# kylejckson/PaintFE

Measured on AMD Instinct MI355X. Metric: Mpixels/sec: 8K 32-layer flatten + Gaussian sigma=16; HBM GB/s vs peak, higher is better.
Workload: dtype f32 (Gaussian leg: f16 taps x u8, f32 accumulate)

## Files before the change

paintfe_amd/csrc/k_flatten.hip:

```cpp
#include <algorithm>
#include <atomic>
#include <type_traits>
#include "k_common.h"
#include "pfx_kernels.h"

using namespace pfxk;

#include "k_blend.h"

typedef float pfx_v4f __attribute__((ext_vector_type(4)));
typedef int pfx_v4i __attribute__((ext_vector_type(4)));
__device__ pfx_v4f pfx_buffer_load_format_v4f32(pfx_v4i rsrc, int voffset, int soffset, int aux) __asm("llvm.amdgcn.raw.buffer.load.format.v4f32");
__device__ float pfx_buffer_load_format_f32(pfx_v4i rsrc, int voffset, int soffset, int aux) __asm("llvm.amdgcn.raw.buffer.load.format.f32");
__device__ void pfx_buffer_store_i32(int data, pfx_v4i rsrc, int voffset, int soffset, int aux) __asm("llvm.amdgcn.raw.buffer.store.i32");
__device__ void pfx_buffer_store_format_v4f32(pfx_v4f data, pfx_v4i rsrc, int voffset, int soffset, int aux) __asm("llvm.amdgcn.raw.buffer.store.format.v4f32");


namespace {


PFX_DEV uint32_t apply_conceal(uint32_t px, uint32_t conceal)
{
    if (conceal == 0u) return px;
    uint32_t a = ((px >> 24) * (255u - conceal)) / 255u;
// ... 464 lines not shown
                    }
                }
                if (lane == 0) { rec[u % NREC][0] = r; rec[u % NREC][1] = best != 0u ? q_tail : 0u; }
                wave_lds_sync();
                cls_next = u + 1u;
                continue;
            }
            if (q_cnt == 0u) {
                if (lane == 0 && (C.stats & 1u)) {
                    atomicAdd(&g_dle_stats[0], st_rounds); atomicAdd(&g_dle_stats[1], st_rpx); atomicAdd(&g_dle_stats[2], st_rlay);
                    atomicAdd(&g_dle_stats[3], nat_next); atomicAdd(&g_dle_stats[4], st_nlay); atomicAdd(&g_dle_stats[5], st_reads);
                    atomicAdd(&g_dle_stats[6], st_cunits);
                }
                break;
            }
            run_queue = true;
        }

        int voff[PX];
        float acc[PX][4];
        uint32_t lb, le;
        if (run_queue) {
            const uint32_t m = min(q_cnt, UPX);
#pragma unroll
            for (int j = 0; j < PX; ++j) {
                const uint32_t k = 64u * j + lane;
                const uint32_t o = (uint32_t)q[(q_head + k) % QCAP];
                voff[j] = k < m ? (int)((base_px + o) * 4u) : (int)bytes;
                acc[j][0] = acc[j][1] = acc[j][2] = acc[j][3] = 0.0f;
            }
            lb = q_start; le = q_r;
            q_head += m;
            st_rounds += 1u; st_rpx += m; st_rlay += le - lb;
        } else {
            const uint32_t o0 = nat_next * UPX + lane;
#pragma unroll
            for (int j = 0; j < PX; ++j) {
                voff[j] = (int)((base_px + o0 + 64u * j) * 4u);
                const uint32_t p = acc_ring[(o0 + 64u * j) % RING];
                acc[j][0] = div255(ubyte0(p)); acc[j][1] = div255(ubyte1(p)); acc[j][2] = div255(ubyte2(p)); acc[j][3] = div255(ubyte3(p));
            }
            lb = nat_start; le = n_layers;
            st_nlay += le - lb;
        }
        dle_layers<PX, NB, AUX>(acc, layers, lb, le, bytes, voff, (C.stats & 2u) != 0u);
#pragma unroll
        for (int j = 0; j < PX; ++j) {
            const uint32_t px = (uint32_t)(acc[j][0] * 255.0f + 0.5f) | ((uint32_t)(acc[j][1] * 255.0f + 0.5f) << 8) |
                                ((uint32_t)(acc[j][2] * 255.0f + 0.5f) << 16) | ((uint32_t)(acc[j][3] * 255.0f + 0.5f) << 24);
            if (run_queue) { if (voff[j] != (int)bytes) acc_ring[((uint32_t)voff[j] / 4u - base_px) % RING] = px; }
            else pfx_buffer_store_i32((int)px, rs_dst, voff[j], 0, 0);
        }
        if (run_queue) wave_lds_sync();
        else nat_next += 1u;
    }
}


#ifndef PFX_SRT_GROUPS
#define PFX_SRT_GROUPS 1
#endif
#ifndef PFX_SRT_REDEAL
#define PFX_SRT_REDEAL 1
#endif
#ifndef PFX_SRT_TYPED_STORE
#define PFX_SRT_TYPED_STORE 0
#endif
#ifndef PFX_SRT_NATSTORE
#define PFX_SRT_NATSTORE 1
#endif
template <int PX>
PFX_DEV void stream_layer_groups(float (&acc)[PX][4], const float (&t)[PX][4], uint32_t mode, float opacity, uint32_t lead)
{
    const float amax = alpha_max<PX>(t);
#if PFX_TWO_STAGE
    if (__any(amax != 0.0f)) blend_layer_nx_two_stage<PX>(mode, acc, t, opacity, lead);
#elif PFX_SRT_GROUPS
    if (__any(amax != 0.0f)) blend_layer_nx_groups<PX>(mode, acc, t, opacity, lead);
#else
    if (__any(amax != 0.0f)) blend_layer_nx<PX>(mode, acc, t, opacity);
#endif
}

template <int PX, bool NOBLEND = false, bool TR = false>
PFX_DEV void srt_layers(float (&acc)[PX][4], const pfxk_layer_desc* __restrict__ layers, uint32_t lb, uint32_t le, uint32_t bytes, int (&voff)[PX],
                        uint32_t s1, uint32_t seg, float4* s_x, uint32_t* s_v, uint32_t& st_moves, unsigned long long* tr = nullptr)
{
    float t[2][PX][4];
    uint32_t m[2], o[2];
    const pfxk_layer_desc* nptr = layers + lb;
    pfxk_layer_desc nd = *nptr;
    uint32_t next_attempt = lb < s1 ? s1 : lb + 1u;
    uint32_t lead = 0u;
    bool recount = true;
    auto fetch = [&](auto SET) {
        constexpr int S = decltype(SET)::value;
        m[S] = nd.mode; o[S] = nd.adj_off;
        const pfx_v4i rs = make_rsrc_canonical(nd.pixels, bytes, PFX_RSRC_UNORM8X4);
#pragma unroll
        for (int j = 0; j < PX; ++j) {
            const pfx_v4f v = pfx_buffer_load_format_v4f32(rs, voff[j], 0, 0);
            t[S][j][0] = v.x; t[S][j][1] = v.y; t[S][j][2] = v.z; t[S][j][3] = v.w;
        }
        nptr += 1;
        nd = *nptr;
    };
    auto blend = [&](auto SET, uint32_t K) {
        constexpr int S = decltype(SET)::value;
        if (K < le) {
            unsigned long long c0 = 0, c1 = 0;
            if constexpr (TR) {
                c0 = __builtin_amdgcn_s_memtime();
                if constexpr (PX == 1) asm volatile("s_waitcnt vmcnt(1)" ::: "memory");
                else if constexpr (PX == 2) asm volatile("s_waitcnt vmcnt(2)" ::: "memory");
                else asm volatile("s_waitcnt vmcnt(3)" ::: "memory");
                c1 = __builtin_amdgcn_s_memtime();
                tr[0] += c1 - c0;
            }
            if constexpr (NOBLEND) {
#pragma unroll
                for (int j = 0; j < PX; ++j) { acc[j][0] += t[S][j][0]; acc[j][1] += t[S][j][1]; acc[j][2] += t[S][j][2]; acc[j][3] = t[S][j][3]; }
            } else if constexpr (PX == 1 && !PFX_TWO_STAGE) {
                stream_layer<1>(acc, t[S], m[S], __builtin_bit_cast(float, __builtin_amdgcn_readfirstlane(o[S])));
            } else {
                if (recount) { lead = count_lead<PX>(acc); recount = false; }
                stream_layer_groups<PX>(acc, t[S], m[S], __builtin_bit_cast(float, __builtin_amdgcn_readfirstlane(o[S])), lead);
                recount = m[S] == M_XOR || m[S] == M_OVERWRITE;
            }
            if constexpr (TR) {
                float sink = 0.0f;
#pragma unroll
                for (int j = 0; j < PX; ++j) sink += acc[j][0] + acc[j][3];
                asm volatile("" :: "v"(sink));
                tr[1] += __builtin_amdgcn_s_memtime() - c1;
            }
        }
    };
    auto redeal = [&](auto SET, uint32_t K) {
        constexpr int S = decltype(SET)::value;
#if !PFX_SRT_REDEAL
        return;
#endif
        if constexpr (PX == 1 || NOBLEND) return;
        if (K != next_attempt || K >= le) return;
        next_attempt = K + seg;
        uint64_t mo[PX];
        uint32_t co[PX], total_o = 0u, now = 0u;
        bool run = true;
#pragma unroll
        for (int j = 0; j < PX; ++j) {
            mo[j] = __ballot(acc[j][3] == 1.0f);
            co[j] = (uint32_t)__popcll(mo[j]);
            total_o += co[j];
            run = run && co[j] == 64u;
            now += run ? 1u : 0u;
        }
        lead = now; recount = false;
        if (total_o / 64u <= now) return;
        lead = total_o / 64u;
        const uint32_t lane = __builtin_amdgcn_mbcnt_hi(~0u, __builtin_amdgcn_mbcnt_lo(~0u, 0u));
        uint32_t slot[PX], pre_o = 0u, pre_n = total_o;
#pragma unroll
        for (int j = 0; j < PX; ++j) {
            const uint32_t rank_o = __builtin_amdgcn_mbcnt_hi((uint32_t)(mo[j] >> 32), __builtin_amdgcn_mbcnt_lo((uint32_t)mo[j], 0u));
            slot[j] = acc[j][3] == 1.0f ? pre_o + rank_o : pre_n + (lane - rank_o);
            pre_o += co[j]; pre_n += 64u - co[j];
        }
#pragma unroll
        for (int j = 0; j < PX; ++j) { s_x[slot[j]] = make_float4(acc[j][0], acc[j][1], acc[j][2], acc[j][3]); s_v[slot[j]] = (uint32_t)voff[j]; }
        wave_lds_sync();
#pragma unroll
        for (int j = 0; j < PX; ++j) {
            const float4 a = s_x[64u * j + lane];
            acc[j][0] = a.x; acc[j][1] = a.y; acc[j][2] = a.z; acc[j][3] = a.w;
            voff[j] = (int)s_v[64u * j + lane];
        }
        wave_lds_sync();
#pragma unroll
        for (int j = 0; j < PX; ++j) s_x[slot[j]] = make_float4(t[S][j][0], t[S][j][1], t[S][j][2], t[S][j][3]);
        wave_lds_sync();
#pragma unroll
        for (int j = 0; j < PX; ++j) {
            const float4 a = s_x[64u * j + lane];
            t[S][j][0] = a.x; t[S][j][1] = a.y; t[S][j][2] = a.z; t[S][j][3] = a.w;
        }
        wave_lds_sync();
        st_moves += 1u;
    };
    fetch(std::integral_constant<int, 0>{});
    for (uint32_t li = lb; li < le; li += 2) {
        fetch(std::integral_constant<int, 1>{}); blend(std::integral_constant<int, 0>{}, li); redeal(std::integral_constant<int, 1>{}, li + 1);
        fetch(std::integral_constant<int, 0>{}); blend(std::integral_constant<int, 1>{}, li + 1); redeal(std::integral_constant<int, 0>{}, li + 2);
    }
}

template <int NB, bool NOBLEND = false, bool TR = false>
PFX_DEV void srt_early(float (&acc)[1][4], const pfxk_layer_desc* __restrict__ layers, uint32_t lb, uint32_t le, uint32_t bytes, int voff, unsigned long long* tr = nullptr)
{
    static_assert(NB >= 2 && 2 * NB - 2 < PFXK_DESC_PAD, "descriptor padding");
    float t[NB][1][4];
    uint32_t m[NB], o[NB];
    const pfxk_layer_desc* nptr = layers + lb;
    pfxk_layer_desc nd = *nptr;
    uint32_t lead = 0u;
    bool recount = true;
    auto fetch = [&](auto SET) {
        constexpr int S = decltype(SET)::value;
        m[S] = nd.mode; o[S] = nd.adj_off;
        const pfx_v4i rs = make_rsrc_canonical(nd.pixels, bytes, PFX_RSRC_UNORM8X4);
        const pfx_v4f v = pfx_buffer_load_format_v4f32(rs, voff, 0, 0);
        t[S][0][0] = v.x; t[S][0][1] = v.y; t[S][0][2] = v.z; t[S][0][3] = v.w;
        nptr += 1;
        nd = *nptr;
    };
    auto blend = [&](auto SET, uint32_t K) {
        constexpr int S = decltype(SET)::value;
        if (K < le) {
            unsigned long long c0 = 0, c1 = 0;
            if constexpr (TR) {
                c0 = __builtin_amdgcn_s_memtime();
                asm volatile("s_waitcnt vmcnt(%0)" :: "n"(NB - 1) : "memory");
                c1 = __builtin_amdgcn_s_memtime();
                tr[0] += c1 - c0;
            }
            if constexpr (NOBLEND) { acc[0][0] += t[S][0][0]; acc[0][1] += t[S][0][1]; acc[0][2] += t[S][0][2]; acc[0][3] = t[S][0][3]; }
            else {
                if (recount) { lead = count_lead<1>(acc); recount = false; }
                stream_layer_groups<1>(acc, t[S], m[S], __builtin_bit_cast(float, __builtin_amdgcn_readfirstlane(o[S])), lead);
                recount = true;
            }
            if constexpr (TR) {
                const float sink = acc[0][0] + acc[0][3];
                asm volatile("" :: "v"(sink));
                tr[1] += __builtin_amdgcn_s_memtime() - c1;
            }
        }
    };
    auto seq = [&](auto self, auto I, uint32_t li) {
        constexpr int i = decltype(I)::value;
        if constexpr (i < NB) {
            fetch(std::integral_constant<int, (i + NB - 1) % NB>{});
            blend(std::integral_constant<int, i>{}, li + (uint32_t)i);
            self(self, std::integral_constant<int, i + 1>{}, li);
        }
    };
    auto pre = [&](auto self, auto I) {
        constexpr int i = decltype(I)::value;
        if constexpr (i < NB - 1) { fetch(std::integral_constant<int, i>{}); self(self, std::integral_constant<int, i + 1>{}); }
    };
    pre(pre, std::integral_constant<int, 0>{});
    for (uint32_t li = lb; li < le; li += (uint32_t)NB) seq(seq, std::integral_constant<int, 0>{}, li);
}
#ifndef PFX_EARLY_NB
#define PFX_EARLY_NB 2
#endif

struct dle_plan { uint32_t s1, seg; };

#ifndef PFX_SRT_PRIO
#define PFX_SRT_PRIO 0
#endif
#ifndef PFX_SRT_WAVES
#define PFX_SRT_WAVES 8
#endif
#if PFX_SRT_WAVES == 8
#define PFX_SRT_ATTR __attribute__((amdgpu_waves_per_eu(8, 8)))
#elif PFX_SRT_WAVES == 7
#define PFX_SRT_ATTR __attribute__((amdgpu_waves_per_eu(7, 7)))
#else
#define PFX_SRT_ATTR
#endif
template <int PX, bool NOBLEND = false, bool TR = false>
__global__ __launch_bounds__(64) PFX_SRT_ATTR void flatten_srt_kernel(const pfxk_layer_desc* __restrict__ layers, uint32_t n_layers, uint32_t n_px,
                                                                         uint8_t* __restrict__ dst, const pfxk_dle_cands C, const dle_sched SC,
                                                                         const dle_plan P)
{
    constexpr uint32_t UPX = 64u * PX;
    __shared__ float4 s_x[UPX];
    __shared__ uint32_t s_v[UPX];
    soft_d_fill(threadIdx.x, 64u);
    __syncthreads();
    const uint32_t lane = threadIdx.x & 63u;
    const uint32_t gw = __builtin_amdgcn_readfirstlane(blockIdx.x);
    const uint32_t units_total = (n_px + UPX - 1u) / UPX;
    uint32_t u0, U;
    if (gw < SC.wavesA) { U = SC.UA; u0 = gw * SC.UA; }
    else if (gw < SC.wavesA + SC.wavesB) { U = SC.UB; u0 = SC.wavesA * SC.UA + (gw - SC.wavesA) * SC.UB; }
    else { U = SC.UC; u0 = SC.wavesA * SC.UA + SC.wavesB * SC.UB + (gw - SC.wavesA - SC.wavesB) * SC.UC; }
    if (u0 >= units_total) return;
    const uint32_t nu = min(U, units_total - u0);
    const uint32_t base_px = u0 * UPX;
    const uint32_t bytes = n_px * 4u;
#if PFX_SRT_TYPED_STORE
    const pfx_v4i rs_acc = make_rsrc(dst, bytes, PFX_RSRC_UNORM8X4);
#else
    const pfx_v4i rs_dst = make_rsrc(dst, bytes, PFX_RSRC_RAW32);
#endif
    const uint32_t s1 = P.seg != 0u ? P.s1 : 0xFFFFFFFFu;
    uint32_t st_egroups = 0, st_elay = 0, st_nlay = 0, st_reads = 0, st_cunits = 0, st_moves = 0;
    uint32_t probe_fail = 0, skip_left = 0;
    unsigned long long tph[8] = {0, 0, 0, 0, 0, 0, 0, 0}, tc0 = 0;
    const unsigned long long t_birth = TR ? __builtin_amdgcn_s_memtime() : 0ull;
    for (uint32_t u = 0; u < nu; ++u) {
        if constexpr (TR) tc0 = __builtin_amdgcn_s_memtime();
        int voff[PX];
        float acc[PX][4];
#pragma unroll
        for (int j = 0; j < PX; ++j) {
            voff[j] = (int)((base_px + u * UPX + 64u * j + lane) * 4u);
            acc[j][0] = acc[j][1] = acc[j][2] = acc[j][3] = 0.0f;
        }
        uint32_t cls[PX];
#pragma unroll
        for (int j = 0; j < PX; ++j) cls[j] = 0u;
        const bool probe = skip_left == 0u;
        if (!probe) skip_left -= 1u;
        bool done = !probe;
#pragma unroll
        for (int i = 3; i >= 0; --i) {
            if ((uint32_t)i < C.n && !done) {
                const pfx_v4i ra = make_rsrc(layers[C.layer[i]].pixels, bytes, PFX_RSRC_ALPHA8);
                bool all_found = true;
#pragma unroll
                for (int j = 0; j < PX; ++j) {
                    const float a = pfx_buffer_load_format_f32(ra, voff[j], 0, 0);
                    const bool hit = C.kind[i] ? (a == 1.0f) : (a != 0.0f);
                    cls[j] = (cls[j] == 0u && hit) ? (uint32_t)(i + 1) : cls[j];
                    all_found = all_found && cls[j] != 0u;
                }
                done = __all(all_found);
                st_reads += 1u;
            }
        }
        uint32_t cn[5] = {UPX, 0u, 0u, 0u, 0u};
#pragma unroll
        for (int i = 1; i <= 4; ++i)
#pragma unroll
            for (int j = 0; j < PX; ++j) cn[i] += (uint32_t)__popcll(__ballot(cls[j] >= (uint32_t)i));
        uint32_t cmin = 0;
#pragma unroll
        for (int i = 1; i <= 4; ++i) if (cn[i] == UPX) cmin = (uint32_t)i;
        const uint32_t lay[5] = {0u, C.layer[0], C.layer[1], C.layer[2], C.layer[3]};
        uint32_t s_u = 0;
#pragma unroll
        for (int i = 1; i <= 4; ++i) if (cmin == (uint32_t)i) s_u = lay[i];
        uint32_t best = 0, best_sav = 0, r = s_u, eg = 0, cn_best = 0;
#pragma unroll
        for (int i = 1; i <= 4; ++i) {
            if ((uint32_t)i > cmin && (uint32_t)i <= C.n) {
                const uint32_t g = (UPX - cn[i] + 63u) / 64u;
                const uint32_t sav = ((uint32_t)PX - g) * (lay[i] - s_u);
                if (sav > best_sav) { best_sav = sav; best = (uint32_t)i; r = lay[i]; eg = g; cn_best = cn[i]; }
            }
        }
        if (probe) {
            if (best != 0u || s_u != 0u) probe_fail = 0u;
            else if (++probe_fail >= 2u) { probe_fail = 0u; skip_left = 14u; }
        }
        if constexpr (TR) { const unsigned long long c = __builtin_amdgcn_s_memtime(); tph[0] += c - tc0; tc0 = c; }
        if (best != 0u) {
            st_cunits += 1u;
            uint32_t pre_e = 0u, pre_l = UPX - cn_best;
#pragma unroll
            for (int j = 0; j < PX; ++j) {
                const bool early = cls[j] < best;
                const uint64_t m = __ballot(early);
                const uint32_t rank_e = __builtin_amdgcn_mbcnt_hi((uint32_t)(m >> 32), __builtin_amdgcn_mbcnt_lo((uint32_t)m, 0u));
                const uint32_t c = (uint32_t)__popcll(m);
                s_v[early ? pre_e + rank_e : pre_l + (lane - rank_e)] = (uint32_t)voff[j];
                pre_e += c; pre_l += 64u - c;
            }
            wave_lds_sync();
#pragma unroll
            for (int j = 0; j < PX; ++j) voff[j] = (int)s_v[64u * j + lane];
            wave_lds_sync();
            for (uint32_t g = 0; g < eg; ++g) {
                int v1[1];
                float a1[1][4] = {{0.0f, 0.0f, 0.0f, 0.0f}};
                v1[0] = voff[0];
#pragma unroll
                for (int j = 1; j < PX; ++j) v1[0] = g == (uint32_t)j ? voff[j] : v1[0];
                uint32_t none = 0u;
#if PFX_SRT_PRIO
                __builtin_amdgcn_s_setprio(PFX_SRT_PRIO & 3);
#endif
#if PFX_EARLY_NB > 0
                (void)none;
                srt_early<PFX_EARLY_NB, NOBLEND, TR>(a1, layers, s_u, r, bytes, v1[0], tph + 4);
#else
                srt_layers<1, NOBLEND, TR>(a1, layers, s_u, r, bytes, v1, 0xFFFFFFFFu, 0u, s_x, s_v, none, tph + 4);
#endif
#pragma unroll
                for (int j = 0; j < PX; ++j)
                    if (g == (uint32_t)j) { acc[j][0] = a1[0][0]; acc[j][1] = a1[0][1]; acc[j][2] = a1[0][2]; acc[j][3] = a1[0][3]; }
            }
            st_egroups += eg; st_elay += eg * (r - s_u);
        }
        st_nlay += n_layers - r;
        const uint32_t moves_before = st_moves;
        if constexpr (TR) { const unsigned long long c = __builtin_amdgcn_s_memtime(); tph[1] += c - tc0; tc0 = c; }
#if PFX_SRT_PRIO
        __builtin_amdgcn_s_setprio((PFX_SRT_PRIO >> 2) & 3);
#endif
        srt_layers<PX, NOBLEND, TR>(acc, layers, r, n_layers, bytes, voff, s1, P.seg, s_x, s_v, st_moves, tph + 6);
        if constexpr (TR) { const unsigned long long c = __builtin_amdgcn_s_memtime(); tph[2] += c - tc0; tc0 = c; }
        if (PFX_SRT_NATSTORE && (best != 0u || st_moves != moves_before)) {
            const uint32_t ub = (base_px + u * UPX) * 4u;
#pragma unroll
            for (int j = 0; j < PX; ++j) s_x[((uint32_t)voff[j] - ub) >> 2] = make_float4(acc[j][0], acc[j][1], acc[j][2], acc[j][3]);
            wave_lds_sync();
#pragma unroll
            for (int j = 0; j < PX; ++j) {
                const float4 a = s_x[64u * j + lane];
                acc[j][0] = a.x; acc[j][1] = a.y; acc[j][2] = a.z; acc[j][3] = a.w;
                voff[j] = (int)(ub + (64u * j + lane) * 4u);
            }
            wave_lds_sync();
        }
#pragma unroll
        for (int j = 0; j < PX; ++j) {
#if PFX_SRT_TYPED_STORE
            pfx_v4f v; v.x = acc[j][0]; v.y = acc[j][1]; v.z = acc[j][2]; v.w = acc[j][3];
            pfx_buffer_store_format_v4f32(v, rs_acc, voff[j], 0, 0);
#else
            uint32_t px = 0u;
#pragma unroll
            for (int c = 0; c < 4; ++c) px = __builtin_amdgcn_cvt_pk_u8_f32(acc[j][c] * 255.0f, c, px);
            pfx_buffer_store_i32((int)px, rs_dst, voff[j], 0, 0);
#endif
        }
        if constexpr (TR) { const unsigned long long c = __builtin_amdgcn_s_memtime(); tph[3] += c - tc0; tc0 = c; }
    }
    if constexpr (TR) {
        if (lane == 0) {
#pragma unroll
            for (int i = 0; i < 8; ++i) atomicAdd(&g_dle_stats[8 + i], tph[i]);
            atomicAdd(&g_dle_stats[0], __builtin_amdgcn_s_memtime() - t_birth);
            atomicAdd(&g_dle_stats[1], 1ull);
        }
        return;
    }
    if (lane == 0 && (C.stats & 1u)) {
        atomicAdd(&g_dle_stats[0], st_egroups); atomicAdd(&g_dle_stats[1], st_egroups * 64u); atomicAdd(&g_dle_stats[2], st_elay);
        atomicAdd(&g_dle_stats[3], nu); atomicAdd(&g_dle_stats[4], st_nlay); atomicAdd(&g_dle_stats[5], st_reads);
        atomicAdd(&g_dle_stats[6], st_cunits); atomicAdd(&g_dle_stats[7], st_moves);
    }
}

__global__ __launch_bounds__(1024) void dle_probe_kernel(const pfxk_layer_desc* __restrict__ layers, uint32_t cand_layer, uint32_t cand_kind, uint32_t n_px,
                                                         uint32_t* __restrict__ verdict_pinned, uint32_t tag)
{
    __shared__ uint32_t s_cnt;
    if (threadIdx.x == 0) s_cnt = 0u;
    __syncthreads();
    const uint32_t lane = threadIdx.x & 63u, wave = threadIdx.x >> 6;
    const uint32_t units = (n_px + 191u) / 192u, bytes = n_px * 4u;
    const pfx_v4i ra = make_rsrc(layers[cand_layer].pixels, bytes, PFX_RSRC_ALPHA8);
    uint32_t good = 0u;
#pragma unroll 4
    for (uint32_t k = 0; k < 16u; ++k) {
        const uint32_t u = (uint32_t)(((uint64_t)(wave * 16u + k) * units) / 256u);
        bool all_hit = true;
#pragma unroll
        for (uint32_t j = 0; j < 3u; ++j) {
            const uint32_t px = u * 192u + 64u * j + lane;
            const float a = pfx_buffer_load_format_f32(ra, (int)(px * 4u), 0, 0);
            all_hit = all_hit && (px >= n_px || (cand_kind ? (a == 1.0f) : (a != 0.0f)));
        }
        good += __all(all_hit) ? 1u : 0u;
    }
    if (lane == 0) atomicAdd(&s_cnt, good);
    __syncthreads();
    if (threadIdx.x == 0) *verdict_pinned = tag | (s_cnt * 2u >= 256u ? 0x80000000u : 0u);
}

__global__ __launch_bounds__(256) void unorm_store_check_kernel(uint8_t* __restrict__ scratch , unsigned long long* out)
{
    const uint32_t k = threadIdx.x;
    const float bn = div255((float)k);
    const pfx_v4i rs = make_rsrc(scratch, 1024u, PFX_RSRC_UNORM8X4);
    pfx_v4f v; v.x = bn; v.y = div255((float)(255u - k)); v.z = div255((float)((k * 7u) & 255u)); v.w = bn;
    pfx_buffer_store_format_v4f32(v, rs, (int)(k * 4u), 0, 0);
    __syncthreads();
    const uint32_t raw = reinterpret_cast<const volatile uint32_t*>(scratch)[k];
    const uint32_t want = k | ((255u - k) << 8) | (((k * 7u) & 255u) << 16) | (k << 24);
    const pfx_v4f b = pfx_buffer_load_format_v4f32(rs, (int)(k * 4u), 0, 0);
    const bool ok = raw == want && __builtin_bit_cast(uint32_t, b.x) == __builtin_bit_cast(uint32_t, v.x) &&
// ... 336 lines not shown
```

paintfe_amd/csrc/pfx_api.cpp:

```cpp
#include <algorithm>
#include <cmath>
#include <cstring>
#include <vector>

#include "k_brush_math.h"
#include "pfx_internal.h"

void pfx_host_brush_lut(float size, float hardness, bool anti_aliased, uint8_t lut[256]);
void pfx_host_line_points(float x0, float y0, float x1, float y1, uint32_t w, uint32_t h, std::vector<float>& out);
void pfx_host_rhai_levels_lut(float in_black, float in_white, float gamma, uint8_t lut[256]);

static_assert((int)PFX_OP_COUNT == (int)PFXK_OP_COUNT && (int)PFX_OP_DESATURATE == (int)PFXK_OP_DESATURATE, "op ids out of sync");
static_assert((int)PFX_RHAI_COUNT == (int)PFXK_RHAI_COUNT && (int)PFX_RHAI_LEVELS == (int)PFXK_RHAI_LEVELS, "rhai ids out of sync");
static_assert((int)PFX_ADJ_CHANNEL_MIXER == (int)PFXK_ADJ_CHANNEL_MIXER, "layer kinds out of sync");

namespace {

inline size_t img_bytes(uint32_t w, uint32_t h) { return (size_t)w * h * 4; }

inline bool opacity_allows_fast_div(float opacity) { return opacity >= 9.094947017729282e-13f;  }

int check_img(pfx_ctx* ctx, const void* src, const void* dst, uint32_t w, uint32_t h, const char* who)
{
    if (!ctx) return PFX_ERR_INVALID;
// ... 31 lines not shown
{
    PFX_TRY(pfx_reserve(ctx, ctx->st_in, img_bytes(w, h)));
    PFX_TRY(pfx_reserve(ctx, ctx->st_out, img_bytes(w, h)));
    PFX_TRY(pfx_h2d(ctx, ctx->st_in.p, src, img_bytes(w, h)));
    *d_mask = nullptr;
    if (mask) {
        PFX_TRY(pfx_reserve(ctx, ctx->st_mask, (size_t)w * h));
        PFX_TRY(pfx_h2d(ctx, ctx->st_mask.p, mask, (size_t)w * h));
        *d_mask = ctx->st_mask.p;
    }
    return PFX_OK;
}

int finish_out(pfx_ctx* ctx, uint8_t* dst, uint32_t w, uint32_t h)
{
    PFX_TRY(pfx_d2h(ctx, dst, ctx->st_out.p, img_bytes(w, h)));
    return pfx_sync(ctx);
}

int prepare_adjust(pfx_ctx* ctx, int op, const float* p, uint32_t n, pfxk_params& P, bool& needs_lut)
{
    std::memset(&P, 0, sizeof P);
    needs_lut = false;
    auto need = [&](uint32_t k) { return n >= k && p != nullptr; };
    switch (op) {
    case PFX_OP_INVERT: case PFX_OP_INVERT_ALPHA: case PFX_OP_SEPIA: case PFX_OP_DESATURATE: return PFX_OK;
    case PFX_OP_BRIGHTNESS_CONTRAST:
        if (!need(2)) break;
        P.p[0] = p[0]; P.p[1] = pfx_host_bc_factor(p[1]); return PFX_OK;
    case PFX_OP_HSL:
        if (!need(3)) break;
        P.p[0] = p[0] / 360.0f;
        P.p[1] = 1.0f + p[1] / 100.0f;
        P.p[2] = p[2] * 255.0f / 100.0f;
        P.p[11] = (std::isfinite(P.p[0]) && std::isfinite(P.p[1]) && std::isfinite(P.p[2])) ? 1.0f : 0.0f;
        return PFX_OK;
    case PFX_OP_EXPOSURE:
        if (!need(1)) break;
        P.p[0] = pfx_host_exposure_gain(p[0]); return PFX_OK;
    case PFX_OP_HIGHLIGHTS_SHADOWS:
        if (!need(2)) break;
        P.p[0] = p[0] / 100.0f; P.p[1] = p[1] / 100.0f; return PFX_OK;
    case PFX_OP_TEMPERATURE_TINT:
        if (!need(2)) break;
        P.p[0] = p[0] * 1.5f; P.p[1] = p[1] * 1.0f; return PFX_OK;
    case PFX_OP_THRESHOLD:
        if (!need(1)) break;
        P.p[0] = p[0]; return PFX_OK;
    case PFX_OP_POSTERIZE:
        if (!need(1)) break;
        P.p[0] = std::max(p[0], 2.0f); return PFX_OK;
    case PFX_OP_COLOR_BALANCE:
        if (!need(9)) break;
        for (int i = 0; i < 9; ++i) P.p[i] = p[i];
        return PFX_OK;
    case PFX_OP_BLACK_AND_WHITE:
        if (!need(3)) break;
        P.p[0] = p[0]; P.p[1] = p[1]; P.p[2] = p[2]; return PFX_OK;
    case PFX_OP_VIBRANCE:
        if (!need(1)) break;
        P.p[0] = p[0] / 100.0f;
        P.p[11] = std::isfinite(P.p[0]) ? 1.0f : 0.0f;
        return PFX_OK;
    case PFX_OP_GRADIENT_MAP: case PFX_OP_LUT_RGBA: needs_lut = true; return PFX_OK;
    default: return pfx_fail(ctx, PFX_ERR_INVALID, "pfx_adjust: unknown op %d", op);
    }
    return pfx_fail(ctx, PFX_ERR_INVALID, "pfx_adjust: op %d needs more parameters (got %u)", op, n);
}

int upload_lut(pfx_ctx* ctx, const uint8_t* lut_host, size_t bytes)
{
    uint8_t padded[1024] = {0};
    std::memcpy(padded, lut_host, std::min<size_t>(bytes, 1024));
    PFX_TRY(pfx_reserve(ctx, ctx->d_lut, 1024));
    return pfx_h2d(ctx, ctx->d_lut.p, padded, 1024);
}

struct preview_arg {
    const void* d_pixels = nullptr;
    const void* d_chunk_present = nullptr;
    pfx_preview info{};
};

int build_stack(pfx_ctx* ctx, const void* const* layer_ptrs, const void* const* mask_ptrs, const pfx_layer_info* layers,
                uint32_t n, uint32_t w, uint32_t h, bool from_store, uint32_t* n_desc, bool* general, bool* has_adj,
                uint32_t track_info = 0xFFFFFFFFu, uint32_t* track_pos = nullptr, const uint8_t** track_pixels = nullptr,
                pfxk_dle_cands* cands = nullptr, std::vector<uint8_t>* chunk_meta = nullptr, bool* shallow = nullptr)
{
    std::vector<const uint8_t*> flag_ptrs;
    std::vector<pfxk_layer_desc> desc;
    std::vector<float> adj;
    desc.reserve(n);
    *general = false;
    *has_adj = false;
    if (track_pos) *track_pos = 0xFFFFFFFFu;
    for (uint32_t i = 0; i < n; ++i) {
        const pfx_layer_info& L = layers[i];
        if (!L.visible) continue;
        pfxk_layer_desc d{};
        d.opacity = L.opacity;
        d.mode = L.blend_mode > 24 ? 0u : (uint32_t)L.blend_mode;
        d.kind = L.kind;
        if (L.kind != PFX_LAYER_RASTER) {
            if (L.kind > PFX_ADJ_CHANNEL_MIXER) return pfx_fail(ctx, PFX_ERR_INVALID, "layer %u: unknown kind %u", i, L.kind);
            d.adj_off = (uint32_t)adj.size();
            float a[16];
            std::memcpy(a, L.adj, sizeof a);
            if (L.kind == PFX_ADJ_EXPOSURE) a[0] = pfx_host_exposure_gain(L.adj[0]);
            if (L.kind == PFX_ADJ_BRIGHTNESS_CONTRAST) a[1] = pfx_host_bc_factor(L.adj[1]);
            adj.insert(adj.end(), a, a + 16);
            *general = true;
            *has_adj = true;
        } else if (from_store) {
            auto it = ctx->layers.find(L.layer_idx);
            if (it == ctx->layers.end()) continue;
            if (it->second.w != w || it->second.h != h)
                return pfx_fail(ctx, PFX_ERR_INVALID, "layer %u is %ux%u, canvas is %ux%u", L.layer_idx, it->second.w, it->second.h, w, h);
            d.pixels = (const uint8_t*)it->second.pixels.p;
            if (it->second.has_mask) { d.mask = (const uint8_t*)it->second.mask.p; *general = true; }
            flag_ptrs.resize(desc.size() + 1, nullptr);
            flag_ptrs[desc.size()] = it->second.has_mask ? nullptr : (const uint8_t*)it->second.chunk_flags.p;
        } else {
            d.pixels = (const uint8_t*)layer_ptrs[i];
            if (!d.pixels) return pfx_fail(ctx, PFX_ERR_INVALID, "layer %u: null device pointer", i);
            if (mask_ptrs && mask_ptrs[i]) { d.mask = (const uint8_t*)mask_ptrs[i]; *general = true; }
        }
        if (d.kind == PFX_LAYER_RASTER) {
            const float c = d.opacity < 0.0f ? 0.0f : (d.opacity > 1.0f ? 1.0f : d.opacity);
            std::memcpy(&d.adj_off, &c, 4);
        }
        if (i == track_info && track_pos && d.kind == PFX_LAYER_RASTER) { *track_pos = (uint32_t)desc.size(); *track_pixels = d.pixels; }
        desc.push_back(d);
    }
    *n_desc = (uint32_t)desc.size();
    if (chunk_meta) {
        chunk_meta->clear();
        flag_ptrs.resize(desc.size(), nullptr);
        std::vector<uint8_t> want(desc.size(), 0);
        bool any = false;
        for (size_t p = 1; p < desc.size(); ++p) {
            if (desc[p].kind != PFX_LAYER_RASTER || desc[p].mask || !flag_ptrs[p]) continue;
            if (desc[p].mode == 14u) want[p] = 2;
            else if (desc[p].mode == 0u && desc[p].opacity >= 1.0f) want[p] = 1;
            any = any || want[p] != 0;
        }
        if (any) {
            chunk_meta->resize(desc.size() * sizeof(void*) + desc.size());
            std::memcpy(chunk_meta->data(), flag_ptrs.data(), desc.size() * sizeof(void*));
            std::memcpy(chunk_meta->data() + desc.size() * sizeof(void*), want.data(), desc.size());
        }
    }
    {
        static const uint8_t cls_of_mode[25] = {2, 2, 1, 2, 0, 0, 0, 0, 1, 2, 1, 2, 2, 0, 2, 1, 0, 1, 2, 0, 2, 0, 1, 0, 1};
        int cls = 2;
        for (const pfxk_layer_desc& d : desc) cls = std::min(cls, d.kind == PFX_LAYER_RASTER && d.mode < 25u ? (int)cls_of_mode[d.mode] : 0);
        ctx->stack_mode_class = desc.empty() ? 0 : cls;
    }
    if (cands) {
        std::memset(cands, 0, sizeof *cands);
        std::vector<std::pair<uint32_t, uint32_t>> found;
        for (uint32_t p = 1; p < desc.size(); ++p) {
            const pfxk_layer_desc& d = desc[p];
            if (d.kind != PFX_LAYER_RASTER || d.mask) continue;
            if (d.mode == 14u) found.emplace_back(p, 0u);
            else if (d.mode == 0u && d.opacity >= 1.0f) found.emplace_back(p, 1u);
        }
        if (desc.size() < (size_t)ctx->dle_min_layers) { if (shallow && ctx->dle_adaptive) *shallow = true; else found.clear(); }
        const size_t kmax = std::min<size_t>(PFXK_DLE_MAX, std::max<size_t>(1, desc.size() / 6));
        const size_t first = found.size() > kmax ? found.size() - kmax : 0;
        for (size_t k = first; k < found.size(); ++k) {
            cands->layer[cands->n] = found[k].first;
            cands->kind[cands->n] = found[k].second;
            cands->n++;
        }
    }
    if (!desc.empty()) { const pfxk_layer_desc last = desc.back(); desc.insert(desc.end(), PFXK_DESC_PAD, last); }
    const size_t desc_bytes = desc.size() * sizeof(pfxk_layer_desc), adj_bytes = adj.size() * sizeof(float);
    const bool same_desc = ctx->d_desc.p && ctx->desc_cache.size() == desc_bytes && (desc_bytes == 0 || std::memcmp(ctx->desc_cache.data(), desc.data(), desc_bytes) == 0);
    if (!same_desc) {
        ctx->desc_cache.clear();
        PFX_TRY(pfx_reserve(ctx, ctx->d_desc, std::max<size_t>(desc.size(), 1) * sizeof(pfxk_layer_desc)));
        PFX_TRY(pfx_h2d(ctx, ctx->d_desc.p, desc.data(), desc_bytes));
        ctx->desc_cache.assign((const uint8_t*)desc.data(), (const uint8_t*)desc.data() + desc_bytes);
    }
    if (!adj.empty()) {
        const bool same_adj = ctx->d_adj.p && ctx->adj_cache.size() == adj_bytes && std::memcmp(ctx->adj_cache.data(), adj.data(), adj_bytes) == 0;
        if (!same_adj) {
            ctx->adj_cache.clear();
            PFX_TRY(pfx_reserve(ctx, ctx->d_adj, adj_bytes));
            PFX_TRY(pfx_h2d(ctx, ctx->d_adj.p, adj.data(), adj_bytes));
            ctx->adj_cache.assign((const uint8_t*)adj.data(), (const uint8_t*)adj.data() + adj_bytes);
        }
    }
    return PFX_OK;
}

int flatten_common(pfx_ctx* ctx, const void* const* layer_ptrs, const void* const* mask_ptrs, const pfx_layer_info* layers,
                   uint32_t n_layers, uint32_t w, uint32_t h, bool from_store, void* dst_dev, const preview_arg* pv = nullptr,
                   const pfxk_region* region = nullptr, const uint8_t* chunk_keys_host = nullptr)
{
    PFX_REQUIRE(ctx, n_layers <= PFX_MAX_LAYERS, "too many layers");
    PFX_REQUIRE(ctx, n_layers == 0 || layers, "null layer list");
    if (!from_store && layer_ptrs && dst_dev)
        for (uint32_t l = 0; l < n_layers; ++l)
            if (layer_ptrs[l] && layer_ptrs[l] != dst_dev && ranges_overlap(layer_ptrs[l], dst_dev, img_bytes(w, h)))
                return pfx_fail(ctx, PFX_ERR_INVALID, "pfx_flatten_dev: dst partially overlaps layer %u (it may be a layer, or disjoint from all)", l);
    uint32_t n_desc = 0, active_pos = 0xFFFFFFFFu;
    const uint8_t* active_pixels = nullptr;
    bool general = false, has_adj = false;
    pfxk_dle_cands cands{};
    std::vector<uint8_t> chunk_meta;
    bool shallow = false;
    PFX_TRY(build_stack(ctx, layer_ptrs, mask_ptrs, layers, n_layers, w, h, from_store, &n_desc, &general, &has_adj,
                        pv ? pv->info.active_layer : 0xFFFFFFFFu, &active_pos, &active_pixels, &cands, from_store ? &chunk_meta : nullptr,
                        from_store ? nullptr : &shallow));
    bool probe_now = false;
    uint32_t probe_layer = 0, probe_kind = 0;
    if (shallow && cands.n > 0) {
        const bool usable = !general && !region && !(pv && pv->d_pixels) && (uint64_t)w * h < (1ull << 30);
        std::vector<uint8_t> key(ctx->desc_cache);
        key.insert(key.end(), (const uint8_t*)&w, (const uint8_t*)&w + 4); key.insert(key.end(), (const uint8_t*)&h, (const uint8_t*)&h + 4);
        const bool same = ctx->dle_probe_state != 0 && key == ctx->dle_probe_key;
        if (same && ctx->dle_probe_state == 1 && hipEventQuery(ctx->ev_dle_probe) == hipSuccess)
            ctx->dle_probe_state = *ctx->h_dle_verdict == (ctx->dle_probe_tag | 0x80000000u) ? 2 : 3;
        if (usable && !same) { probe_now = true; ctx->dle_probe_key.swap(key); ctx->dle_probe_state = 0; }
        probe_layer = cands.layer[cands.n - 1u]; probe_kind = cands.kind[cands.n - 1u];
        if (!(usable && same && ctx->dle_probe_state == 2)) cands.n = 0;
    }
    const size_t nchunks = (size_t)((w + 63) / 64) * ((h + 63) / 64);
    uint8_t* d_chunks = nullptr;
    bool chunks_ready = false;
    if (has_adj) {
        PFX_TRY(pfx_reserve(ctx, ctx->d_chunks, nchunks));
        d_chunks = (uint8_t*)ctx->d_chunks.p;
        if (chunk_keys_host && !(pv && pv->d_pixels)) { PFX_TRY(pfx_h2d(ctx, d_chunks, chunk_keys_host, nchunks)); chunks_ready = true; }
    }
    pfxk_preview PV{};
    if (pv && pv->d_pixels) {
        PFX_TRY(pfx_reserve(ctx, ctx->fx_a, 2 * nchunks));
        uint8_t* flags = (uint8_t*)ctx->fx_a.p;
        if (pv->d_chunk_present) PFX_HIP(ctx, hipMemcpyAsync(flags, pv->d_chunk_present, nchunks, hipMemcpyDeviceToDevice, ctx->stream));
        else PFX_HIP(ctx, pfxk_chunk_populated(ctx->stream, (const uint8_t*)pv->d_pixels, w, h, flags));
        if (active_pixels) PFX_HIP(ctx, pfxk_chunk_populated(ctx->stream, active_pixels, w, h, flags + nchunks));
        PV.pixels = (const uint8_t*)pv->d_pixels;
        PV.chunk_present = flags;
        PV.layer_chunk_present = flags + nchunks;
        PV.active_pos = active_pos;
        PV.mode = pv->info.blend_mode > 24 ? 0u : pv->info.blend_mode;
        PV.is_eraser = pv->info.is_eraser != 0;
        PV.replaces = pv->info.replaces_layer != 0;
    }
    bool fast_div = true;
    for (uint32_t i = 0; i < n_layers; ++i) fast_div = fast_div && opacity_allows_fast_div(layers[i].opacity);
    const uint8_t* d_chunk_start = nullptr;
    if (ctx->use_chunk_start && !chunk_meta.empty() && !general && fast_div && !region && !PV.pixels && cands.n == 0 && n_desc < 255) {
        if (!ctx->h_chunk_useful) {
            PFX_HIP(ctx, hipHostMalloc((void**)&ctx->h_chunk_useful, sizeof(uint32_t), hipHostMallocDefault));
            *ctx->h_chunk_useful = 0;
            PFX_HIP(ctx, hipEventCreateWithFlags(&ctx->ev_chunk_useful, hipEventDisableTiming));
// ... 1293 lines not shown
```

paintfe_amd/csrc/pfx_kernels.h:

```cpp
#pragma once
#include <hip/hip_runtime.h>
#include <stdint.h>

#ifdef __cplusplus
extern "C" {
#endif

enum { PFXK_LAYER_RASTER = 0, PFXK_ADJ_EXPOSURE = 1, PFXK_ADJ_BRIGHTNESS_CONTRAST = 2, PFXK_ADJ_INVERT = 3,
       PFXK_ADJ_CHANNEL_MIXER = 4 };

typedef struct pfxk_layer_desc {
    const uint8_t* pixels;
    const uint8_t* mask;
    float    opacity;
    uint32_t mode;
    uint32_t kind;
    uint32_t adj_off;
} pfxk_layer_desc;

typedef struct pfxk_params { float p[12]; } pfxk_params;

enum { PFXK_OP_INVERT = 0, PFXK_OP_INVERT_ALPHA, PFXK_OP_SEPIA, PFXK_OP_BRIGHTNESS_CONTRAST, PFXK_OP_HSL,
       PFXK_OP_EXPOSURE, PFXK_OP_HIGHLIGHTS_SHADOWS, PFXK_OP_TEMPERATURE_TINT, PFXK_OP_THRESHOLD, PFXK_OP_POSTERIZE,
       PFXK_OP_COLOR_BALANCE, PFXK_OP_GRADIENT_MAP, PFXK_OP_BLACK_AND_WHITE, PFXK_OP_VIBRANCE, PFXK_OP_LUT_RGBA,
       PFXK_OP_DESATURATE, PFXK_OP_COUNT };
enum { PFXK_RHAI_INVERT = 0, PFXK_RHAI_DESATURATE, PFXK_RHAI_SEPIA, PFXK_RHAI_SEPIA_STRENGTH,
       PFXK_RHAI_BRIGHTNESS_CONTRAST, PFXK_RHAI_HSL, PFXK_RHAI_EXPOSURE, PFXK_RHAI_LEVELS, PFXK_RHAI_COUNT };

typedef struct pfxk_preview {
    const uint8_t* pixels;
    const uint8_t* chunk_present;
    const uint8_t* layer_chunk_present;
    uint32_t active_pos;
    uint32_t mode, is_eraser, replaces;
} pfxk_preview;
typedef struct pfxk_region { uint32_t x0, y0, rw, rh; } pfxk_region;
#define PFXK_DLE_MAX 4
#define PFXK_DESC_PAD 16
typedef struct pfxk_dle_cands { uint32_t n; uint32_t layer[PFXK_DLE_MAX]; uint32_t kind[PFXK_DLE_MAX]; uint32_t stats;  } pfxk_dle_cands;
hipError_t pfxk_flatten(hipStream_t stream, const pfxk_layer_desc* d_layers, uint32_t n_layers,
                        const float* d_adj_table, int general, int fast_div, uint8_t* d_chunk_active, int chunk_active_ready, uint32_t w,
                        uint32_t h, uint8_t* d_dst, const pfxk_preview* preview ,
                        const pfxk_region* region , const pfxk_dle_cands* cands ,
                        const uint8_t* d_chunk_start ,
                        int typed_store_ok ,
                        int mode_class );
hipError_t pfxk_chunk_alpha_flags(hipStream_t s, const uint8_t* d_px, uint32_t w, uint32_t h, uint32_t cx0, uint32_t cy0, uint32_t ncx, uint32_t ncy,
                                  uint8_t* d_flags);
hipError_t pfxk_chunk_start(hipStream_t s, const uint8_t* const* d_flag_ptrs, const uint8_t* d_want, uint32_t n_layers, uint32_t n_chunks,
                            uint8_t* d_start, uint32_t* useful_pinned , uint32_t tag);
void       pfxk_flatten_set_dle(int units_per_wave , int ring_log2 );
hipError_t pfxk_dle_probe(hipStream_t s, const pfxk_layer_desc* d_layers, uint32_t cand_layer, uint32_t cand_kind, uint32_t n_px, uint32_t* verdict_pinned, uint32_t tag);
hipError_t pfxk_flatten_dle_stats(unsigned long long* out16 , int reset);
void       pfxk_flatten_set_dle_dev(int stats_on , int cfg );
void       pfxk_flatten_set_dle_sched(int sched , int fracA, int fracB);
void       pfxk_flatten_set_dle_plan(int kernel , int s1 ,
                                     int s2 );
hipError_t pfxk_unorm_store_check(hipStream_t s, uint8_t* d_scratch1k, unsigned long long* d_out);
void       pfxk_flatten_set_variant(int v);
hipError_t pfxk_rdiv_check(hipStream_t s, uint64_t seed, uint32_t blocks, uint32_t iters, unsigned long long* d_out);
hipError_t pfxk_round_pack_check(hipStream_t s, unsigned long long* d_out );

int        pfxk_gauss_max_radius(void);
int        pfxk_gauss_weight_pad(void);
void       pfxk_gauss_set_v_config(int cfg);
void       pfxk_gauss_set_mfma_segments(int n);
void pfxk_gauss_set_fused_exact(int on);
int pfxk_gauss_fused_exact_max_radius(void);
hipError_t pfxk_gauss_plane_exact(hipStream_t stream, const uint8_t* d_src, uint8_t* d_dst, const float* d_wts_tap0, int radius, uint32_t w, uint32_t h);
hipError_t pfxk_gauss_fused_exact(hipStream_t stream, const uint8_t* d_src, uint8_t* d_dst, const float* d_wts_tap0, int radius, uint32_t w, uint32_t h,
                                  int epilogue , float p0, const uint8_t* d_mask);
hipError_t pfxk_gauss_h(hipStream_t stream, const uint8_t* d_src, float* d_tmp, const float* d_wts_tap0, int radius,
                        uint32_t w, uint32_t h, int exact);
int        pfxk_gauss_mfma_max_radius(void);
int        pfxk_gauss_mfma_wlen(void);
int        pfxk_gauss_mfma_woff(void);
hipError_t pfxk_gauss_mfma(hipStream_t stream, const uint8_t* d_src, uint8_t* d_dst, const uint16_t* d_wsplit,
                           int radius, float inv_scale2, float bias_c, float bias_single, uint32_t w, uint32_t h, uint32_t first_row, int n_cus);
hipError_t pfxk_gauss_mfma_chain(hipStream_t stream, const uint8_t* d_src, uint8_t* d_dst, const uint16_t* d_wsplit, int radius, float inv_scale2, float bias_c,
                                 float bias_single, uint32_t w, uint32_t h, uint32_t first_row, int n_cus, const struct pfxk_chain* chain);
void       pfxk_gauss_set_mfma_cols64(int mask);
void       pfxk_gauss_set_mfma_parts(int weight_parts, int h_parts);
hipError_t pfxk_gauss_v(hipStream_t stream, const float* d_tmp, uint8_t* d_dst, const float* d_wts_tap0, int radius,
                        uint32_t w, uint32_t h, int exact);

#define PFXK_CHAIN_MAX 8
#define PFXK_CHAIN_LUTS 4
#define PFXK_CHAIN_RHAI 0x100u
typedef struct pfxk_chain {
    uint32_t n, n_luts;
    uint32_t op[PFXK_CHAIN_MAX];
    uint32_t lut_slot[PFXK_CHAIN_MAX];
    pfxk_params P[PFXK_CHAIN_MAX];
} pfxk_chain;
hipError_t pfxk_pointwise_chain(hipStream_t s, const uint8_t* d_src, uint8_t* d_dst, const uint8_t* d_luts, const pfxk_chain* C, uint32_t w, uint32_t h);
hipError_t pfxk_gauss_fused_exact_chain(hipStream_t stream, const uint8_t* d_src, uint8_t* d_dst, const float* d_wts_tap0, int radius, uint32_t w, uint32_t h,
                                        const pfxk_chain* C, const uint8_t* d_luts);

hipError_t pfxk_adjust(hipStream_t s, const uint8_t* d_src, uint8_t* d_dst, const uint8_t* d_mask, const uint8_t* d_lut,
                       int op, const pfxk_params* P, int sparse_mode, uint32_t w, uint32_t h);
hipError_t pfxk_rhai_adjust(hipStream_t s, uint8_t* d_px, const uint8_t* d_lut, int op, const pfxk_params* P,
// ... 131 lines not shown
```

Before: 29290.

## Precompute per-layer buffer descriptors and dispatch words on host for streaming flatten

Adds a second descriptor table, appended after the layer descriptors, holding a prebuilt buffer resource, opacity offset and a packed dispatch word with mode, full-opacity and lower-mode flags. The streaming and early-layer loops read this table, so they no longer build the resource descriptor per layer, and they always go through the two-stage blend path keyed by the masked mode. The aim is to cut per-layer scalar overhead in the hot loop. In exchange the descriptor upload grows, the PX==1 single-layer path is removed, and the resource format constant is duplicated, which could drift from the kernel-side definition.

```diff
diff --git a/paintfe_amd/csrc/k_flatten.hip b/paintfe_amd/csrc/k_flatten.hip
--- a/paintfe_amd/csrc/k_flatten.hip
+++ b/paintfe_amd/csrc/k_flatten.hip
@@ -570,21 +570,28 @@
 #endif
 }
 
+template <int PX>
+PFX_DEV void stream_layer_disp(float (&acc)[PX][4], const float (&t)[PX][4], uint32_t disp, float opacity, uint32_t lead)
+{
+    const float amax = alpha_max<PX>(t);
+    if (__any(amax != 0.0f)) blend_layer_nx_two_stage<PX>(disp & 31u, acc, t, opacity, lead);
+}
+
 template <int PX, bool NOBLEND = false, bool TR = false>
-PFX_DEV void srt_layers(float (&acc)[PX][4], const pfxk_layer_desc* __restrict__ layers, uint32_t lb, uint32_t le, uint32_t bytes, int (&voff)[PX],
+PFX_DEV void srt_layers(float (&acc)[PX][4], const pfxk_srt_desc* __restrict__ srt, uint32_t lb, uint32_t le, uint32_t bytes, int (&voff)[PX],
                         uint32_t s1, uint32_t seg, float4* s_x, uint32_t* s_v, uint32_t& st_moves, unsigned long long* tr = nullptr)
 {
     float t[2][PX][4];
     uint32_t m[2], o[2];
-    const pfxk_layer_desc* nptr = layers + lb;
-    pfxk_layer_desc nd = *nptr;
+    const pfxk_srt_desc* nptr = srt + lb;
+    pfxk_srt_desc nd = *nptr;
     uint32_t next_attempt = lb < s1 ? s1 : lb + 1u;
     uint32_t lead = 0u;
     bool recount = true;
     auto fetch = [&](auto SET) {
         constexpr int S = decltype(SET)::value;
-        m[S] = nd.mode; o[S] = nd.adj_off;
-        const pfx_v4i rs = make_rsrc_canonical(nd.pixels, bytes, PFX_RSRC_UNORM8X4);
+        m[S] = nd.disp; o[S] = nd.opc;
+        pfx_v4i rs; rs.x = (int)nd.rsrc[0]; rs.y = (int)nd.rsrc[1]; rs.z = (int)bytes; rs.w = (int)PFXK_RSRC_UNORM8X4;
 #pragma unroll
         for (int j = 0; j < PX; ++j) {
             const pfx_v4f v = pfx_buffer_load_format_v4f32(rs, voff[j], 0, 0);
@@ -608,12 +615,10 @@
             if constexpr (NOBLEND) {
 #pragma unroll
                 for (int j = 0; j < PX; ++j) { acc[j][0] += t[S][j][0]; acc[j][1] += t[S][j][1]; acc[j][2] += t[S][j][2]; acc[j][3] = t[S][j][3]; }
-            } else if constexpr (PX == 1 && !PFX_TWO_STAGE) {
-                stream_layer<1>(acc, t[S], m[S], __builtin_bit_cast(float, __builtin_amdgcn_readfirstlane(o[S])));
             } else {
                 if (recount) { lead = count_lead<PX>(acc); recount = false; }
-                stream_layer_groups<PX>(acc, t[S], m[S], __builtin_bit_cast(float, __builtin_amdgcn_readfirstlane(o[S])), lead);
-                recount = m[S] == M_XOR || m[S] == M_OVERWRITE;
+                stream_layer_disp<PX>(acc, t[S], m[S], __builtin_bit_cast(float, __builtin_amdgcn_readfirstlane(o[S])), lead);
+                recount = (m[S] & PFXK_SRT_LOWER) != 0u;
             }
             if constexpr (TR) {
                 float sink = 0.0f;
@@ -683,19 +688,19 @@
 }
 
 template <int NB, bool NOBLEND = false, bool TR = false>
-PFX_DEV void srt_early(float (&acc)[1][4], const pfxk_layer_desc* __restrict__ layers, uint32_t lb, uint32_t le, uint32_t bytes, int voff, unsigned long long* tr = nullptr)
+PFX_DEV void srt_early(float (&acc)[1][4], const pfxk_srt_desc* __restrict__ srt, uint32_t lb, uint32_t le, uint32_t bytes, int voff, unsigned long long* tr = nullptr)
 {
     static_assert(NB >= 2 && 2 * NB - 2 < PFXK_DESC_PAD, "descriptor padding");
     float t[NB][1][4];
     uint32_t m[NB], o[NB];
-    const pfxk_layer_desc* nptr = layers + lb;
-    pfxk_layer_desc nd = *nptr;
+    const pfxk_srt_desc* nptr = srt + lb;
+    pfxk_srt_desc nd = *nptr;
     uint32_t lead = 0u;
     bool recount = true;
     auto fetch = [&](auto SET) {
         constexpr int S = decltype(SET)::value;
-        m[S] = nd.mode; o[S] = nd.adj_off;
-        const pfx_v4i rs = make_rsrc_canonical(nd.pixels, bytes, PFX_RSRC_UNORM8X4);
+        m[S] = nd.disp; o[S] = nd.opc;
+        pfx_v4i rs; rs.x = (int)nd.rsrc[0]; rs.y = (int)nd.rsrc[1]; rs.z = (int)bytes; rs.w = (int)PFXK_RSRC_UNORM8X4;
         const pfx_v4f v = pfx_buffer_load_format_v4f32(rs, voff, 0, 0);
         t[S][0][0] = v.x; t[S][0][1] = v.y; t[S][0][2] = v.z; t[S][0][3] = v.w;
         nptr += 1;
@@ -714,7 +719,7 @@
             if constexpr (NOBLEND) { acc[0][0] += t[S][0][0]; acc[0][1] += t[S][0][1]; acc[0][2] += t[S][0][2]; acc[0][3] = t[S][0][3]; }
             else {
                 if (recount) { lead = count_lead<1>(acc); recount = false; }
-                stream_layer_groups<1>(acc, t[S], m[S], __builtin_bit_cast(float, __builtin_amdgcn_readfirstlane(o[S])), lead);
+                stream_layer_disp<1>(acc, t[S], m[S], __builtin_bit_cast(float, __builtin_amdgcn_readfirstlane(o[S])), lead);
                 recount = true;
             }
             if constexpr (TR) {
@@ -784,6 +789,7 @@
 #else
     const pfx_v4i rs_dst = make_rsrc(dst, bytes, PFX_RSRC_RAW32);
 #endif
+    const pfxk_srt_desc* const srt = reinterpret_cast<const pfxk_srt_desc*>(layers + n_layers + PFXK_DESC_PAD);
     const uint32_t s1 = P.seg != 0u ? P.s1 : 0xFFFFFFFFu;
     uint32_t st_egroups = 0, st_elay = 0, st_nlay = 0, st_reads = 0, st_cunits = 0, st_moves = 0;
     uint32_t probe_fail = 0, skip_left = 0;
@@ -874,9 +880,9 @@
 #endif
 #if PFX_EARLY_NB > 0
                 (void)none;
-                srt_early<PFX_EARLY_NB, NOBLEND, TR>(a1, layers, s_u, r, bytes, v1[0], tph + 4);
+                srt_early<PFX_EARLY_NB, NOBLEND, TR>(a1, srt, s_u, r, bytes, v1[0], tph + 4);
 #else
-                srt_layers<1, NOBLEND, TR>(a1, layers, s_u, r, bytes, v1, 0xFFFFFFFFu, 0u, s_x, s_v, none, tph + 4);
+                srt_layers<1, NOBLEND, TR>(a1, srt, s_u, r, bytes, v1, 0xFFFFFFFFu, 0u, s_x, s_v, none, tph + 4);
 #endif
 #pragma unroll
                 for (int j = 0; j < PX; ++j)
@@ -890,7 +896,7 @@
 #if PFX_SRT_PRIO
         __builtin_amdgcn_s_setprio((PFX_SRT_PRIO >> 2) & 3);
 #endif
-        srt_layers<PX, NOBLEND, TR>(acc, layers, r, n_layers, bytes, voff, s1, P.seg, s_x, s_v, st_moves, tph + 6);
+        srt_layers<PX, NOBLEND, TR>(acc, srt, r, n_layers, bytes, voff, s1, P.seg, s_x, s_v, st_moves, tph + 6);
         if constexpr (TR) { const unsigned long long c = __builtin_amdgcn_s_memtime(); tph[2] += c - tc0; tc0 = c; }
         if (PFX_SRT_NATSTORE && (best != 0u || st_moves != moves_before)) {
             const uint32_t ub = (base_px + u * UPX) * 4u;
diff --git a/paintfe_amd/csrc/pfx_api.cpp b/paintfe_amd/csrc/pfx_api.cpp
--- a/paintfe_amd/csrc/pfx_api.cpp
+++ b/paintfe_amd/csrc/pfx_api.cpp
@@ -137,6 +137,29 @@
     pfx_preview info{};
 };
 
+}
+extern "C" void pfxk_srt_desc_fill(const pfxk_layer_desc* desc, uint32_t n, uint32_t w, uint32_t h, pfxk_srt_desc* out)
+{
+    if (n == 0) return;
+    const uint32_t bytes = (uint32_t)((size_t)w * h * 4);
+    const uint32_t opaque_below = desc[0].mode == 0u && desc[0].opacity >= 1.0f ? 1u : 0u;
+    uint32_t next = n;
+    for (uint32_t k = n; k-- > 0;) {
+        const pfxk_layer_desc& d = desc[k];
+        const uint32_t mode = d.mode > 24u ? 0u : d.mode;
+        const bool lower = mode == 13u || mode == 14u;
+        if (lower) next = k;
+        const uint64_t a = (uint64_t)(uintptr_t)d.pixels;
+        pfxk_srt_desc& o = out[k];
+        o.rsrc[0] = (uint32_t)a; o.rsrc[1] = (uint32_t)(a >> 32); o.rsrc[2] = bytes; o.rsrc[3] = PFXK_RSRC_UNORM8X4;
+        o.opc = d.adj_off;
+        o.disp = mode | (d.opacity >= 1.0f ? PFXK_SRT_FULL : 0u) | (lower ? PFXK_SRT_LOWER : 0u);
+        o.next_lower = next;
+        o.opaque_below = opaque_below;
+    }
+    for (uint32_t k = n; k < n + PFXK_DESC_PAD; ++k) { out[k] = out[n - 1]; out[k].next_lower = n; }
+}
+namespace {
 int build_stack(pfx_ctx* ctx, const void* const* layer_ptrs, const void* const* mask_ptrs, const pfx_layer_info* layers,
                 uint32_t n, uint32_t w, uint32_t h, bool from_store, uint32_t* n_desc, bool* general, bool* has_adj,
                 uint32_t track_info = 0xFFFFFFFFu, uint32_t* track_pos = nullptr, const uint8_t** track_pixels = nullptr,
@@ -230,6 +253,15 @@
         }
     }
     if (!desc.empty()) { const pfxk_layer_desc last = desc.back(); desc.insert(desc.end(), PFXK_DESC_PAD, last); }
+    static_assert(sizeof(pfxk_srt_desc) == sizeof(pfxk_layer_desc) && sizeof(pfxk_srt_desc) == 32, "the two tables share one array");
+    if (!desc.empty()) {
+        const uint32_t nd = *n_desc;
+        std::vector<pfxk_srt_desc> srt(nd + PFXK_DESC_PAD);
+        pfxk_srt_desc_fill(desc.data(), nd, w, h, srt.data());
+        const size_t at = desc.size();
+        desc.resize(at + srt.size());
+        std::memcpy((void*)(desc.data() + at), srt.data(), srt.size() * sizeof(pfxk_srt_desc));
+    }
     const size_t desc_bytes = desc.size() * sizeof(pfxk_layer_desc), adj_bytes = adj.size() * sizeof(float);
     const bool same_desc = ctx->d_desc.p && ctx->desc_cache.size() == desc_bytes && (desc_bytes == 0 || std::memcmp(ctx->desc_cache.data(), desc.data(), desc_bytes) == 0);
     if (!same_desc) {
diff --git a/paintfe_amd/csrc/pfx_kernels.h b/paintfe_amd/csrc/pfx_kernels.h
--- a/paintfe_amd/csrc/pfx_kernels.h
+++ b/paintfe_amd/csrc/pfx_kernels.h
@@ -17,6 +17,18 @@
     uint32_t kind;
     uint32_t adj_off;
 } pfxk_layer_desc;
+
+#define PFXK_RSRC_UNORM8X4 (0xFACu | (0u << 12) | (10u << 15))
+#define PFXK_SRT_FULL  0x100u
+#define PFXK_SRT_LOWER 0x200u
+typedef struct __attribute__((aligned(32))) pfxk_srt_desc {
+    uint32_t rsrc[4];
+    uint32_t opc;
+    uint32_t disp;
+    uint32_t next_lower;
+    uint32_t opaque_below;
+} pfxk_srt_desc;
+void pfxk_srt_desc_fill(const pfxk_layer_desc* desc, uint32_t n, uint32_t w, uint32_t h, pfxk_srt_desc* out);
 
 typedef struct pfxk_params { float p[12]; } pfxk_params;
 
```

Result: no change. 29290, median of 6 (+0.0%).
